# LeiXu84/fireFoam-dev

Measured on AMD Instinct MI355X. Metric: PIMPLE outer-iterations/sec on 64M-cell hex mesh; pEqn SpMV GB/s vs HBM peak, higher is better.
Workload: dtype f64; 1 GPU; synthetic 400^3 hex box (64000000 cells), buoyant plume + 5-species EDC-shaped source, PIMPLE 1/2/0: rhoEqn + UEqn + YEEqn(4 Yi + h) + 2 pEqn per step; cells=64000000, faces=191520000, parallelism=1 GPU, transport_solvers=PBiCGStab+DILU

## Files before the change

### firefoam-dev_amd/binding.py

```python
import ctypes as C
import os
import re
import subprocess

import numpy as np

_HERE = os.path.dirname(os.path.abspath(__file__))
_ROOT = os.path.dirname(_HERE)
_SO = os.path.join(_HERE, "lib", "libffm.so")
_HDR = os.path.join(_ROOT, "include", "ffm.h")

SOLVERS = {"PCG": 0, "PBiCGStab": 1, "PBiCG": 2, "diagonal": 3, "smoothSolver": 4}
PRECONDS = {"none": 0, "DIC": 1, "DILU": 2, "GaussSeidel": 3, "symGaussSeidel": 4, "diagonal": 5}


class FfmError(RuntimeError):
    pass


class Perf(C.Structure):
    _fields_ = [("initialResidual", C.c_double), ("finalResidual", C.c_double),
                ("nIterations", C.c_int), ("converged", C.c_int), ("singular", C.c_int)]

    def as_dict(self):
# ... 62 lines not shown
        "ffm_renumber_levels": ([C.c_int, C.c_int, ip, ip, ip, ip], C.c_int),
        "ffm_ldu_set_coeffs": ([vp, hp, hp, hp], C.c_int),
        "ffm_ldu_set_coeffs_d": ([vp, dp, dp, dp], C.c_int),
        "ffm_ldu_n_native_faces": ([vp], C.c_int),
        "ffm_ldu_get_face_map": ([vp, ip], C.c_int),
        "ffm_ldu_set_coeffs_native_d": ([vp, dp, dp, dp], C.c_int),
        "ffm_ldu_bind_coeffs_native_d": ([vp, dp, dp, dp, C.c_int], C.c_int),
        "ffm_ldu_set_interfaces": ([vp, C.c_int, ip, C.POINTER(ip), C.POINTER(hp), C.POINTER(hp), ip], C.c_int),
        "ffm_ldu_set_global_cells": ([vp, C.c_long], C.c_int),
        "ffm_spmv": ([vp, dp, dp], C.c_int),
        "ffm_tmul": ([vp, dp, dp], C.c_int),
        "ffm_sumA": ([vp, dp], C.c_int),
        "ffm_residual": ([vp, dp, dp, dp], C.c_int),
        "ffm_precond_setup": ([vp, C.c_int, dp], C.c_int),
        "ffm_precond_apply": ([vp, C.c_int, C.c_int, dp, dp], C.c_int),
        "ffm_gs_smooth": ([vp, C.c_int, C.c_int, dp, dp], C.c_int),
        "ffm_solve_d": ([vp, C.c_int, C.c_int, C.c_double, C.c_double, C.c_int, C.c_int, C.c_int, dp, dp,
                         C.POINTER(Perf)], C.c_int),
        "ffm_solve": ([vp, C.c_int, C.c_int, C.c_double, C.c_double, C.c_int, C.c_int, C.c_int, hp, hp,
                       C.POINTER(Perf)], C.c_int),
        "ffm_solve_multi_d": ([vp, C.c_int, C.c_int, C.c_int, C.c_double, C.c_double, C.c_int, C.c_int, C.POINTER(C.c_void_p), dp, dp,
                               C.POINTER(C.c_void_p), C.POINTER(C.c_void_p), C.POINTER(Perf)], C.c_int),
        "ffm_ldu_unbind_coeffs": ([vp], C.c_int),
        "ffm_bench_spmv": ([vp, dp, dp, C.c_int, hp], C.c_int),
        "ffm_bench_precond": ([vp, C.c_int, dp, dp, C.c_int, hp], C.c_int),
        "ffm_debug_set_sweep_ticket": ([vp, C.c_uint], C.c_int),
        "ffm_ldu_set_exchange_tags": ([vp, C.c_int, C.c_int, ip], C.c_int),
        "ffm_field_binary": ([vp, C.c_int, C.c_long, dp, dp, dp], C.c_int),
        "ffm_field_scalar": ([vp, C.c_int, C.c_long, dp, C.c_double, C.c_int, dp], C.c_int),
        "ffm_field_unary": ([vp, C.c_int, C.c_long, dp, dp], C.c_int),
# ... 430 lines not shown

    def residual(self, psi, source):
        self.ctx._ready()
        r = self.ctx.empty(self.nCells)
        _check(lib().ffm_residual(self.h, C.c_void_p(psi.data_ptr()), C.c_void_p(source.data_ptr()),
                                  C.c_void_p(r.data_ptr())), "ffm_residual")
        self.ctx.sync()
        return r

    def reciprocalD(self, preconditioner):
        rD = self.ctx.empty(self.nCells)
        _check(lib().ffm_precond_setup(self.h, PRECONDS[preconditioner], C.c_void_p(rD.data_ptr())), "ffm_precond_setup")
        self.ctx.sync()
        return rD

    def precondition(self, preconditioner, rA, transpose=False):
        self.ctx._ready()
        w = self.ctx.empty(self.nCells)
        _check(lib().ffm_precond_apply(self.h, PRECONDS[preconditioner], 1 if transpose else 0,
                                       C.c_void_p(rA.data_ptr()), C.c_void_p(w.data_ptr())), "ffm_precond_apply")
        self.ctx.sync()
        return w

    def smooth(self, psi, source, nSweeps=1, smoother="symGaussSeidel"):
        self.ctx._ready()
        psi = psi.clone()
        self.ctx._ready()
        _check(lib().ffm_gs_smooth(self.h, 1 if smoother == "symGaussSeidel" else 0, nSweeps,
                                   C.c_void_p(psi.data_ptr()), C.c_void_p(source.data_ptr())), "ffm_gs_smooth")
        self.ctx.sync()
# ... 414 lines not shown
```

### firefoam-dev_amd/csrc/ffm_solve.hip

```cpp
#include "ffm_internal.hpp"
#include "ffm_device.hpp"
#include <algorithm>
#include <cmath>
#include <cstring>

static inline int sgrid(long n) { long g = (n + 255) / 256; return (int)std::max(1L, std::min(g, (long)RED_BLOCKS)); }

enum {
    OP_XREF = 1, OP_NORMF, OP_RES_INIT, OP_RES, OP_PCG_BETA, OP_PCG_ALPHA,
    OP_BS_RHO, OP_BS_ALPHA, OP_BS_OMEGA, OP_BICG_BETA, OP_BICG_ALPHA, OP_RESET
};

#define VSMALL_ 1e-300

__global__ void k_scalar_op(double *__restrict__ s, int op, double arg, int iter)
{
    if (threadIdx.x || blockIdx.x) return;
    switch (op) {
    case OP_RESET:
        s[S_SING] = 0.0; s[S_WARA] = 1e+20; s[S_WARA_OLD] = 1e+20; s[S_RA0RA] = 0.0; s[S_ALPHA] = 0.0; s[S_OMEGA] = 0.0;
        s[S_BETA] = 0.0;
        break;
    case OP_XREF: s[S_XREF] = s[S_TMP0] / arg; break;
    case OP_NORMF: s[S_NORMF] = s[S_TMP0] + 1e-20; break;
    case OP_RES_INIT: s[S_RES] = s[S_TMP0] / s[S_NORMF]; s[S_RES0] = s[S_RES]; break;
    case OP_RES: if (s[S_SING] == 0.0) s[S_RES] = s[S_TMP0] / s[S_NORMF]; break;
    case OP_PCG_BETA: {
        const double old = s[S_WARA], nw = s[S_TMP0];
        s[S_WARA_OLD] = old; s[S_WARA] = nw; s[S_BETA] = nw / old;
        break; }
    case OP_PCG_ALPHA: case OP_BICG_ALPHA: {
        const double wApA = s[S_TMP0];
        s[S_WAPA] = wApA;
        if (fabs(wApA) / s[S_NORMF] > VSMALL_) { s[S_ALPHA] = s[S_WARA] / wApA; }
        else { s[S_SING] = 1.0; s[S_ALPHA] = 0.0; }
        break; }
    case OP_BS_RHO: {
        const double old = s[S_RA0RA], nw = s[S_TMP0];
        s[S_RA0RA_OLD] = old; s[S_RA0RA] = nw;
        if (!(fabs(nw) > VSMALL_)) { s[S_SING] = 1.0; break; }
        if (iter > 0) {
            if (!(fabs(s[S_OMEGA]) > VSMALL_)) { s[S_SING] = 1.0; break; }
            s[S_BETA] = (nw / old) * (s[S_ALPHA] / s[S_OMEGA]);
        }
        break; }
    case OP_BS_ALPHA: if (s[S_SING] == 0.0) { s[S_RA0AYA] = s[S_TMP0]; s[S_ALPHA] = s[S_RA0RA] / s[S_TMP0]; } break;
    case OP_BS_OMEGA: if (s[S_SING] == 0.0) { s[S_TATA] = s[S_TMP0]; s[S_TASA] = s[S_TMP1]; s[S_OMEGA] = s[S_TMP1] / s[S_TMP0]; } break;
    case OP_BICG_BETA: {
        const double old = s[S_WARA], nw = s[S_TMP0];
        s[S_WARA_OLD] = old; s[S_WARA] = nw; s[S_BETA] = nw / old;
        break; }
    }
}

static int scalar_op(ffm_ctx *c, int op, double arg = 0.0, int iter = 0)
{
    hipLaunchKernelGGL(k_scalar_op, dim3(1), dim3(64), 0, c->stream, c->scal_d, op, arg, iter);
    FFM_HIP(hipGetLastError());
    return FFM_OK;
}
static int finish_dot(ffm_ctx *c, int op, int nSlots = 1, double arg = 0.0, int iter = 0)
{
    if (c->nRanks > 1 || c->comm) FFM_TRY(ffm_allreduce_slots(c, S_TMP0, nSlots));
    return scalar_op(c, op, arg, iter);
}

#define GRID_STRIDE(i, n) for (long i = (long)blockIdx.x * blockDim.x + threadIdx.x; i < (n); i += (long)gridDim.x * blockDim.x)

__global__ void k_sub(long n, double *__restrict__ r, const double *__restrict__ b, const double *__restrict__ w)
{ GRID_STRIDE(i, n) r[i] = b[i] - w[i]; }

__global__ void k_sub2(long n, double *__restrict__ r, double *__restrict__ rT, const double *__restrict__ b,
                       const double *__restrict__ w, const double *__restrict__ wT)
{ GRID_STRIDE(i, n) { r[i] = b[i] - w[i]; rT[i] = b[i] - wT[i]; } }

__global__ void k_copy(long n, double *__restrict__ d, const double *__restrict__ s)
{ GRID_STRIDE(i, n) d[i] = s[i]; }

__global__ __launch_bounds__(256) void k_normf(long n, const double *__restrict__ Ax, const double *__restrict__ b,
                                               const double *__restrict__ sumA, const double *__restrict__ scal,
                                               double *__restrict__ partials)
{
    __shared__ double sm[4];
    const double xRef = scal[S_XREF];
    double acc = 0.0;
    GRID_STRIDE(i, n) { const double t = sumA[i] * xRef; acc += fabs(Ax[i] - t) + fabs(b[i] - t); }
    const double r = block_sum(acc, sm);
    if (threadIdx.x == 0) partials[blockIdx.x] = r;
}

__global__ void k_p_update(long n, double *__restrict__ p, const double *__restrict__ w, const double *__restrict__ scal, int first)
{
    if (scal[S_SING] != 0.0) return;
    const double beta = scal[S_BETA];
    if (first) { GRID_STRIDE(i, n) p[i] = w[i]; }
    else { GRID_STRIDE(i, n) p[i] = w[i] + beta * p[i]; }
}

__global__ void k_p_psi(long n, double *__restrict__ psi, double *__restrict__ p, const double *__restrict__ w, const double *__restrict__ scal)
{
    if (scal[S_SING] != 0.0) return;
    const double alpha = scal[S_ALPHA], beta = scal[S_BETA];
    GRID_STRIDE(i, n) { const double pi = p[i]; psi[i] += alpha * pi; p[i] = w[i] + beta * pi; }
// ... 12 lines not shown
        if (!sing) { psi[i] += alpha * p[i]; ri -= alpha * w[i]; r[i] = ri; }
        acc += fabs(ri);
    }
    const double s = block_sum(acc, sm);
    if (threadIdx.x == 0) partials[blockIdx.x] = s;
}

__global__ void k_axmy_alpha(long n, double *__restrict__ r, const double *__restrict__ w, const double *__restrict__ scal)
{
    if (scal[S_SING] != 0.0) return;
    const double alpha = scal[S_ALPHA];
    GRID_STRIDE(i, n) r[i] -= alpha * w[i];
}

__global__ void k_bs_p(long n, double *__restrict__ p, const double *__restrict__ r, const double *__restrict__ AyA,
                       const double *__restrict__ scal, int first)
{
    if (scal[S_SING] != 0.0) return;
    const double beta = scal[S_BETA], omega = scal[S_OMEGA];
    if (first) { GRID_STRIDE(i, n) p[i] = r[i]; }
    else { GRID_STRIDE(i, n) p[i] = r[i] + beta * (p[i] - omega * AyA[i]); }
}

__global__ __launch_bounds__(256) void k_bs_s(long n, double *__restrict__ sA, const double *__restrict__ r,
                                              const double *__restrict__ AyA, const double *__restrict__ scal,
                                              double *__restrict__ partials)
{
    __shared__ double sm[4];
    const double alpha = scal[S_ALPHA];
    const bool sing = scal[S_SING] != 0.0;
    double acc = 0.0;
    if (!sing) GRID_STRIDE(i, n) { const double v = r[i] - alpha * AyA[i]; sA[i] = v; acc += fabs(v); }
    const double s = block_sum(acc, sm);
    if (threadIdx.x == 0) partials[blockIdx.x] = s;
}

// ... 240 lines not shown
    FFM_HIP(hipMemcpyAsync(h, A->sweepTicket, sizeof(h), hipMemcpyDeviceToHost, A->ctx->stream));
    FFM_HIP(hipStreamSynchronize(A->ctx->stream));
    if (h[1]) {
        ffm_set_error(A->sweepMode == 2 ? "tiled sweep timed out waiting for a value of a predecessor group (abort word set)"
                                        : "dataflow sweep timed out waiting for the value of a predecessor cell (abort word set)");
        unsigned int z = 0;
        ffm_h2d(A->ctx, A->sweepTicket + 1, &z, sizeof(z));
        return FFM_ERR_HIP;
    }
    return FFM_OK;
}

static int calc_rD(ffm_ldu *A)
{
    if (A->sweepMode == 2) {
        FFM_TRY(ffm_tile_calc_rD(A));
        hipLaunchKernelGGL(k_recip, dim3(sgrid(A->nOwned)), dim3(256), 0, A->ctx->stream, (long)A->nOwned, A->rD, A->rD);
        FFM_HIP(hipGetLastError());
        return FFM_OK;
    }
    FlowArgs a; FFM_TRY(flow_args(A, SM_RD, a));
    FLOW_LAUNCH(SM_RD, a);
    FFM_HIP(hipGetLastError());
    return FFM_OK;
}

int ffm_precond_setup_i(ffm_ldu *A, int precond)
{
    if (A->rDKind == precond && A->rDEpoch == A->coeffEpoch) return FFM_OK;
    hipStream_t s = A->ctx->stream;
    switch (precond) {
    case FFM_NONE: break;
    case FFM_DIC:
        if (!A->symmetric) { ffm_set_error("DIC needs a symmetric matrix"); return FFM_ERR_UNSUPPORTED; }
// ... 52 lines not shown
        a.bP = bUse; a.psi = psi;
        if (sym) FLOW_LAUNCH(SM_SYMGS, a); else FLOW_LAUNCH(SM_GS, a);
        FFM_HIP(hipGetLastError());
    }
    return FFM_OK;
}

struct Controls { double tol, relTol; int minIter, maxIter, nSweeps; };

static inline bool check_convergence(ffm_perf *p, const Controls &k)
{
    p->converged = (p->finalResidual < k.tol || (k.relTol > 1e-20 && p->finalResidual < k.relTol * p->initialResidual)) ? 1 : 0;
    return p->converged;
}

static int norm_and_initial(ffm_ldu *A, const double *psi, const double *source, const double *Apsi, double *tmp,
                            const double *rA, ffm_perf *perf)
{
    ffm_ctx *c = A->ctx; hipStream_t s = c->stream; const long N = A->nOwned;
    FFM_TRY(ffm_k_sum(c, psi, N, S_TMP0));
    FFM_TRY(finish_dot(c, OP_XREF, 1, (double)A->globalCells));
    const int g = sgrid(N);
    hipLaunchKernelGGL(k_normf, dim3(g), dim3(256), 0, s, N, Apsi, source, tmp, c->scal_d, c->partials_d);
    FFM_TRY(partial_sum_to(c, g, S_TMP0));
    FFM_TRY(finish_dot(c, OP_NORMF));
    FFM_TRY(ffm_k_summag(c, rA, N, S_TMP0));
    FFM_TRY(finish_dot(c, OP_RES_INIT));
    FFM_TRY(ffm_read_scalars(c));
    perf->initialResidual = c->scal_h[S_RES0];
    perf->finalResidual = perf->initialResidual;
    perf->nIterations = 0; perf->singular = 0; perf->converged = 0;
    return FFM_OK;
}

static int pcg(ffm_ldu *A, int precond, const Controls &k, double *psi, const double *source, ffm_perf *perf)
{
    ffm_ctx *c = A->ctx; hipStream_t s = c->stream; const long N = A->nOwned; const int g = sgrid(N);
    double *pA, *wA, *rA;
    FFM_TRY(ffm_ldu_work(A, 1, &pA)); FFM_TRY(ffm_ldu_work(A, 2, &wA)); FFM_TRY(ffm_ldu_work(A, 3, &rA));
    FFM_TRY(scalar_op(c, OP_RESET));
    FFM_TRY(ffm_k_spmv_sumA(A, psi, wA, pA));
    hipLaunchKernelGGL(k_sub, dim3(g), dim3(256), 0, s, N, rA, source, wA);
    FFM_TRY(norm_and_initial(A, psi, source, wA, pA, rA, perf));
    if (k.minIter > 0 || !check_convergence(perf, k)) {
        FFM_TRY(ffm_precond_setup_i(A, precond));
        if (precond == FFM_DIC && A->sweepMode == 2 && ffm_tile_pcg_fusable(A)) {
            const bool fuseP = ffm_tile_amul_pcg_usable(A);
            double *pB = nullptr, *qA = wA;
            if (fuseP) { FFM_TRY(ffm_ldu_work(A, 4, &pB)); FFM_TRY(ffm_ldu_work(A, 5, &qA)); }
            do {
                if (perf->nIterations == 0) {
                    FFM_TRY(ffm_precond_apply_i(A, precond, false, rA, wA));
                    FFM_TRY(ffm_k_dot(c, wA, rA, N, S_TMP0));
                } else FFM_TRY(ffm_tile_pcg_bwd(A, rA, wA, S_TMP0));
                FFM_TRY(finish_dot(c, OP_PCG_BETA));
                if (perf->nIterations == 0) {
                    hipLaunchKernelGGL(k_p_update, dim3(g), dim3(256), 0, s, N, pA, wA, c->scal_d, 1);
// ... 26 lines not shown
            hipLaunchKernelGGL(k_pcg_xr, dim3(g), dim3(256), 0, s, N, psi, rA, pA, wA, c->scal_d, c->partials_d);
            FFM_TRY(partial_sum_to(c, g, S_TMP0));
            FFM_TRY(finish_dot(c, OP_RES));
            FFM_TRY(ffm_read_scalars(c));
            if (c->scal_h[S_SING] != 0.0) { perf->singular = 1; break; }
            perf->finalResidual = c->scal_h[S_RES];
        } while ((++perf->nIterations < k.maxIter && !check_convergence(perf, k)) || perf->nIterations < k.minIter);
    }
    return FFM_OK;
}

static int pbicgstab(ffm_ldu *A, int precond, const Controls &k, double *psi, const double *source, ffm_perf *perf)
{
    ffm_ctx *c = A->ctx; hipStream_t s = c->stream; const long N = A->nOwned; const int g = sgrid(N);
    double *yA, *rA, *pA, *AyA, *sA, *zA, *tA, *rA0;
    FFM_TRY(ffm_ldu_work(A, 1, &pA)); FFM_TRY(ffm_ldu_work(A, 2, &yA)); FFM_TRY(ffm_ldu_work(A, 3, &rA));
    FFM_TRY(scalar_op(c, OP_RESET));
    FFM_TRY(ffm_k_spmv_sumA(A, psi, yA, pA));
    hipLaunchKernelGGL(k_sub, dim3(g), dim3(256), 0, s, N, rA, source, yA);
    FFM_TRY(norm_and_initial(A, psi, source, yA, pA, rA, perf));
    if (k.minIter > 0 || !check_convergence(perf, k)) {
        FFM_TRY(ffm_ldu_work(A, 4, &AyA)); FFM_TRY(ffm_ldu_work(A, 5, &sA)); FFM_TRY(ffm_ldu_work(A, 6, &zA));
        FFM_TRY(ffm_ldu_work(A, 7, &tA)); FFM_TRY(ffm_ldu_work(A, 8, &rA0));
        hipLaunchKernelGGL(k_copy, dim3(g), dim3(256), 0, s, N, rA0, rA);
        FFM_TRY(ffm_precond_setup_i(A, precond));
        do {
            FFM_TRY(ffm_k_dot(c, rA0, rA, N, S_TMP0));
            FFM_TRY(finish_dot(c, OP_BS_RHO, 1, 0.0, perf->nIterations));
            hipLaunchKernelGGL(k_bs_p, dim3(g), dim3(256), 0, s, N, pA, rA, AyA, c->scal_d, perf->nIterations == 0 ? 1 : 0);
            FFM_TRY(ffm_precond_apply_i(A, precond, false, pA, yA));
            FFM_TRY(ffm_k_spmv(A, yA, AyA, false));
            FFM_TRY(ffm_k_dot(c, rA0, AyA, N, S_TMP0));
            FFM_TRY(finish_dot(c, OP_BS_ALPHA));
            hipLaunchKernelGGL(k_bs_s, dim3(g), dim3(256), 0, s, N, sA, rA, AyA, c->scal_d, c->partials_d);
            FFM_TRY(partial_sum_to(c, g, S_TMP0));
            FFM_TRY(finish_dot(c, OP_RES));
            FFM_TRY(ffm_read_scalars(c));
            if (c->scal_h[S_SING] != 0.0) { perf->singular = 1; break; }
            perf->finalResidual = c->scal_h[S_RES];
            if (check_convergence(perf, k)) {
                hipLaunchKernelGGL(k_axpy_alpha, dim3(g), dim3(256), 0, s, N, psi, yA, c->scal_d);
                perf->nIterations++;
                return FFM_OK;
            }
// ... 9 lines not shown
            perf->finalResidual = c->scal_h[S_RES];
        } while ((++perf->nIterations < k.maxIter && !check_convergence(perf, k)) || perf->nIterations < k.minIter);
    }
    return FFM_OK;
}

static int pbicg(ffm_ldu *A, int precond, const Controls &k, double *psi, const double *source, ffm_perf *perf)
{
    ffm_ctx *c = A->ctx; hipStream_t s = c->stream; const long N = A->nOwned; const int g = sgrid(N);
    double *pA, *pT, *wA, *wT, *rA, *rT;
    FFM_TRY(ffm_ldu_work(A, 1, &pA)); FFM_TRY(ffm_ldu_work(A, 2, &wA)); FFM_TRY(ffm_ldu_work(A, 3, &rA));
    FFM_TRY(ffm_ldu_work(A, 4, &pT)); FFM_TRY(ffm_ldu_work(A, 5, &wT)); FFM_TRY(ffm_ldu_work(A, 6, &rT));
    FFM_TRY(scalar_op(c, OP_RESET));
    FFM_TRY(ffm_k_spmv_sumA(A, psi, wA, pA));
    FFM_TRY(ffm_k_spmv(A, psi, wT, true));
    hipLaunchKernelGGL(k_sub2, dim3(g), dim3(256), 0, s, N, rA, rT, source, wA, wT);
    FFM_TRY(norm_and_initial(A, psi, source, wA, pA, rA, perf));
    if (k.minIter > 0 || !check_convergence(perf, k)) {
        FFM_TRY(ffm_precond_setup_i(A, precond));
        do {
            FFM_TRY(ffm_precond_apply_i(A, precond, false, rA, wA));
            FFM_TRY(ffm_precond_apply_i(A, precond, true, rT, wT));
            FFM_TRY(ffm_k_dot(c, wA, rT, N, S_TMP0));
            FFM_TRY(finish_dot(c, OP_BICG_BETA));
            const int first = perf->nIterations == 0 ? 1 : 0;
            hipLaunchKernelGGL(k_p_update, dim3(g), dim3(256), 0, s, N, pA, wA, c->scal_d, first);
            hipLaunchKernelGGL(k_p_update, dim3(g), dim3(256), 0, s, N, pT, wT, c->scal_d, first);
            FFM_TRY(ffm_k_spmv(A, pA, wA, false));
            FFM_TRY(ffm_k_spmv(A, pT, wT, true));
            FFM_TRY(ffm_k_dot(c, wA, pT, N, S_TMP0));
            FFM_TRY(finish_dot(c, OP_BICG_ALPHA));
            hipLaunchKernelGGL(k_axmy_alpha, dim3(g), dim3(256), 0, s, N, rT, wT, c->scal_d);
            hipLaunchKernelGGL(k_pcg_xr, dim3(g), dim3(256), 0, s, N, psi, rA, pA, wA, c->scal_d, c->partials_d);
            FFM_TRY(partial_sum_to(c, g, S_TMP0));
            FFM_TRY(finish_dot(c, OP_RES));
            FFM_TRY(ffm_read_scalars(c));
            if (c->scal_h[S_SING] != 0.0) { perf->singular = 1; break; }
            perf->finalResidual = c->scal_h[S_RES];
        } while ((++perf->nIterations < k.maxIter && !check_convergence(perf, k)) || perf->nIterations < k.minIter);
    }
    return FFM_OK;
}

static int smooth(ffm_ldu *A, int smoother, const Controls &k, double *psi, const double *source, ffm_perf *perf)
{
    if (smoother != FFM_GS && smoother != FFM_SYMGS) { ffm_set_error("smoothSolver: smoother must be GaussSeidel or symGaussSeidel"); return FFM_ERR_UNSUPPORTED; }
    ffm_ctx *c = A->ctx; hipStream_t s = c->stream; const long N = A->nOwned; const int g = sgrid(N);
    const int nSweeps = k.nSweeps > 0 ? k.nSweeps : 1;
    double *Apsi, *tmp, *res;
    FFM_TRY(ffm_ldu_work(A, 1, &Apsi)); FFM_TRY(ffm_ldu_work(A, 2, &tmp)); FFM_TRY(ffm_ldu_work(A, 3, &res));
    FFM_TRY(scalar_op(c, OP_RESET));
    FFM_TRY(ffm_k_spmv_sumA(A, psi, Apsi, tmp));
    hipLaunchKernelGGL(k_sub, dim3(g), dim3(256), 0, s, N, res, source, Apsi);
    FFM_TRY(norm_and_initial(A, psi, source, Apsi, tmp, res, perf));
    if (k.minIter > 0 || !check_convergence(perf, k)) {
        do {
            FFM_TRY(ffm_gs_smooth_i(A, smoother == FFM_SYMGS, nSweeps, psi, source));
            FFM_TRY(ffm_k_residual(A, psi, source, res));
            FFM_TRY(ffm_k_summag(c, res, N, S_TMP0));
            FFM_TRY(finish_dot(c, OP_RES));
            FFM_TRY(ffm_read_scalars(c));
            perf->finalResidual = c->scal_h[S_RES];
        } while (((perf->nIterations += nSweeps) < k.maxIter && !check_convergence(perf, k)) || perf->nIterations < k.minIter);
    }
    return FFM_OK;
}

static int diagonal(ffm_ldu *A, double *psi, const double *source, ffm_perf *perf)
// ... 89 lines not shown
    if (m == 1) { G.use(L[only]); return ffm_k_spmv(A, L[only].*in, L[only].*out, false); }
    return FFM_OK;
}
static int pbicgstab_multi(ffm_ldu *A, int precond, const Controls &k, int n, Lane *L)
{
    ffm_ctx *c = A->ctx; hipStream_t s = c->stream; const long N = A->nOwned; const int g = sgrid(N);
    LaneGuard G(A);
    {
        const double *dg[FFM_TILE_MAXSYS], *x[FFM_TILE_MAXSYS]; double *y[FFM_TILE_MAXSYS], *sm[FFM_TILE_MAXSYS];
        for (int i = 0; i < n; i++) { dg[i] = L[i].diag; x[i] = L[i].psi; y[i] = L[i].yA; sm[i] = L[i].pA; }
        FFM_TRY(ffm_k_spmv_multi(A, n, dg, x, y, sm));
    }
    for (int i = 0; i < n; i++) {
        Lane &l = L[i]; G.use(l);
        FFM_TRY(scalar_op(c, OP_RESET));
        hipLaunchKernelGGL(k_sub, dim3(g), dim3(256), 0, s, N, l.rA, l.source, l.yA);
        FFM_TRY(norm_and_initial(A, l.psi, l.source, l.yA, l.pA, l.rA, l.perf));
        l.active = k.minIter > 0 || !check_convergence(l.perf, k);
        if (l.active) hipLaunchKernelGGL(k_copy, dim3(g), dim3(256), 0, s, N, l.rA0, l.rA);
    }
    {
        const double *dg[FFM_TILE_MAXSYS]; double *D[FFM_TILE_MAXSYS]; int m = 0, only = -1;
        for (int i = 0; i < n; i++) if (L[i].active) { dg[m] = L[i].diag; D[m] = L[i].rD; m++; only = i; }
        if (m >= 2) {
            FFM_TRY(ffm_tile_calc_rD_multi(A, m, dg, D));
            for (int j = 0; j < m; j++) hipLaunchKernelGGL(k_recip, dim3(g), dim3(256), 0, s, N, D[j], (const double *)D[j]);
        } else if (m == 1) { G.use(L[only]); A->rDKind = -1; FFM_TRY(ffm_precond_setup_i(A, precond)); }
        A->rDKind = precond; A->rDEpoch = A->coeffEpoch;
    }
    for (;;) {
        bool any = false;
        for (int i = 0; i < n; i++) if (L[i].active) {
            Lane &l = L[i]; G.use(l); any = true;
            FFM_TRY(ffm_k_dot(c, l.rA0, l.rA, N, S_TMP0));
            FFM_TRY(finish_dot(c, OP_BS_RHO, 1, 0.0, l.perf->nIterations));
            hipLaunchKernelGGL(k_bs_p, dim3(g), dim3(256), 0, s, N, l.pA, l.rA, l.AyA, c->scal_d, l.perf->nIterations == 0 ? 1 : 0);
        }
        if (!any) break;
        FFM_TRY(precond_lanes(A, precond, L, n, &Lane::pA, &Lane::yA, G));
        FFM_TRY(amul_lanes(A, L, n, &Lane::yA, &Lane::AyA, G));
        for (int i = 0; i < n; i++) if (L[i].active) {
            Lane &l = L[i]; G.use(l);
            FFM_TRY(ffm_k_dot(c, l.rA0, l.AyA, N, S_TMP0));
            FFM_TRY(finish_dot(c, OP_BS_ALPHA));
            hipLaunchKernelGGL(k_bs_s, dim3(g), dim3(256), 0, s, N, l.sA, l.rA, l.AyA, c->scal_d, c->partials_d);
            FFM_TRY(partial_sum_to(c, g, S_TMP0));
            FFM_TRY(finish_dot(c, OP_RES));
        }
        FFM_TRY(read_lane_scalars(c, L, n));
        for (int i = 0; i < n; i++) if (L[i].active) {
            Lane &l = L[i]; G.use(l);
// ... 76 lines not shown
    const size_t nb = sizeof(double) * (size_t)std::max(A->nCells, 1);
    FFM_HIP(hipMalloc((void **)&p, nb)); FFM_HIP(hipMalloc((void **)&b, nb));
    FFM_TRY(ffm_h2d(A->ctx, p, psi, sizeof(double) * A->nOwned));
    FFM_TRY(ffm_h2d(A->ctx, b, source, sizeof(double) * A->nOwned));
    int rc = ffm_solve_d(A, solver, precond, tol, relTol, minIter, maxIter, nSweeps, p, b, out);
    if (!rc) rc = ffm_d2h(A->ctx, psi, p, sizeof(double) * A->nOwned);
    hipFree(p); hipFree(b);
    return rc;
}

extern "C" int ffm_precond_setup(ffm_ldu *A, int precond, double *rD_out_d)
{
    if (!A) return FFM_ERR_ARG;
    FFM_TRY(ffm_precond_setup_i(A, precond));
    if (rD_out_d) FFM_TRY(ffm_from_internal(A, A->rD, rD_out_d));
    FFM_HIP(hipStreamSynchronize(A->ctx->stream));
    FFM_TRY(ffm_sweep_check_abort(A));
    return FFM_OK;
}

extern "C" int ffm_bench_precond(ffm_ldu *A, int precond, const double *r_d, double *w_d, int reps, double *avg_ms)
{
    if (!A || !r_d || !w_d || reps < 1 || !avg_ms) return FFM_ERR_ARG;
    if (!A->identity) { ffm_set_error("ffm_bench_precond needs an LDU in the library's cell order"); return FFM_ERR_UNSUPPORTED; }
    FFM_TRY(ffm_precond_setup_i(A, precond));
    FFM_TRY(ffm_precond_apply_i(A, precond, false, r_d, w_d));
    hipEvent_t e0, e1;
    FFM_HIP(hipEventCreate(&e0)); FFM_HIP(hipEventCreate(&e1));
    FFM_HIP(hipEventRecord(e0, A->ctx->stream));
    for (int i = 0; i < reps; i++) FFM_TRY(ffm_precond_apply_i(A, precond, false, r_d, w_d));
// ... 40 lines not shown
```

### firefoam-dev_amd/csrc/ffm_tile.hip

```cpp
#include "ffm_internal.hpp"
#include "ffm_device.hpp"
#include <algorithm>
#include <atomic>
#include <climits>

constexpr int T_RING = 4096;
constexpr int T_ENT = 256;
constexpr int T_THREADS = 256;
constexpr int T_W = 3;
constexpr int T_PF = 8;
constexpr int T_PM = 3;
constexpr int T_XMAX = 64;
constexpr int T_RINGD = T_RING - 2 * T_ENT;
constexpr unsigned T_SPIN_LIMIT = 1u << 22;
constexpr unsigned T_NONE = 0xFFFFu;
constexpr int T_LDS = T_RING + 2 * T_XMAX + 1;
constexpr unsigned long long T_SENT = 0x7FF4DEADBEEFCAFEull;
static_assert(T_LDS < (int)T_NONE && T_ENT <= 256, "neighbour codes are LDS slots");
static_assert(T_PM >= 2 && T_PM < T_PF, "read-ahead distances");

struct TileDir {
    int nEnt = 0, nPub = 0;
    int *grpEnt = nullptr;
    int4 *rec = nullptr;
// ... 447 lines not shown
                    for (int s = 0; s < W; s++) { const double nv = val - pa[k][s] * pb[k][TWO ? s : 0] / x[s]; val = (cd[s] != T_NONE) ? nv : val; }
                } else if (MODE == TM_GSF) {
                    val = pv[k];
#pragma unroll
                    for (int s = 0; s < W; s++) { const double nv = val - pa[k][s] * x[s]; val = (cd[s] != T_NONE) ? nv : val; }
                    if (pok[k]) *(double *)((char *)aux + c * 8u) = val;
#pragma unroll
                    for (int s = 0; s < W; s++) val -= pb[k][TWO ? s : 0];
                    val = val / d;
                } else {
                    val = pv[k];
#pragma unroll
                    for (int s = 0; s < W; s++) { const double nv = val - pa[k][s] * x[s]; val = (cd[s] != T_NONE) ? nv : val; }
                    val = val / d;
                }
                if (pok[k]) { *(double *)((char *)w + c * 8u) = val; ring[(c - gs) & (unsigned)(T_RING - 1)] = val; }
                if (FUSE && MODE == TM_BWD) fsum += pok[k] ? val * pv2[FUSE ? k : 0] : 0.0;
                if (pok[k] && cd[3] != T_NONE) t_st(&t.mail[ppb[k] + cd[3]], val);
            }
            T_FETCH(k, ee + T_PF, Rn);
            t_barrier();
        }
    }
#undef T_FETCH
    if (FUSE) {
        double v = fsum;
#pragma unroll
        for (int o = 32; o > 0; o >>= 1) v += __shfl_down(v, o, 64);
        if ((tid & 63u) == 0u) shSum[tid >> 6] = v;
        t_barrier();
        if (tid == 0) partials[g] = ((shSum[0] + shSum[1]) + shSum[2]) + shSum[3];
// ... 247 lines not shown
                        for (int s = 0; s < W; s++) { const double nv = v - d * pa[k][s] * ring[i][sl[s]]; v = (cd[s] != T_NONE) ? nv : v; }
                    } else if (MODE == TM_BWD) {
                        v = pv[k][TWO ? 0 : i];
#pragma unroll
                        for (int s = W - 1; s >= 0; s--) { const double nv = v - d * pa[k][s] * ring[i][sl[s]]; v = (cd[s] != T_NONE) ? nv : v; }
                    } else {
                        v = d;
#pragma unroll
                        for (int s = 0; s < W; s++) { const double nv = v - pa[k][s] * pb[k][TWO ? s : 0] / ring[i][sl[s]]; v = (cd[s] != T_NONE) ? nv : v; }
                    }
                    val[i] = v;
                }
                if (pok[k]) {
#pragma unroll
                    for (int i = 0; i < NF; i++) {
                        *(double *)((char *)m.w[i] + c * 8u) = val[i];
                        ring[i][(c - gs) & (unsigned)(T_RING - 1)] = val[i];
                        if (cd[3] != T_NONE) t_st(&m.mail[i][ppb[k] + cd[3]], val[i]);
                    }
                }
            }
            TM_FETCH(k, ee + PF, Rn);
            t_barrier();
        }
    }
#undef TM_FETCH
}


bool ffm_tile_multi_usable(const ffm_ldu *A) { return ffm_tile_usable(A); }
static int tile_multi_mail(ffm_ldu *A)
// ... 308 lines not shown
```

### include/ffm.h

```cpp
#ifndef FFM_H
#define FFM_H

#include <stddef.h>
#include <stdint.h>

#ifdef __cplusplus
extern "C" {
#endif

typedef struct ffm_ctx ffm_ctx;
typedef struct ffm_ldu ffm_ldu;

typedef enum ffm_status {
    FFM_OK = 0,
    FFM_ERR_ARG = -1,
    FFM_ERR_ADDR = -2,
    FFM_ERR_HIP = -3,
    FFM_ERR_NODEVICE = -4,
    FFM_ERR_UNSUPPORTED = -5,
    FFM_ERR_COMM = -6
} ffm_status;

typedef enum ffm_solver {
    FFM_PCG = 0, FFM_PBICGSTAB = 1, FFM_PBICG = 2, FFM_DIAGONAL = 3, FFM_SMOOTH = 4,
// ... 81 lines not shown
int ffm_ldu_set_interfaces(ffm_ldu *ldu, int nPatches, const int *patchSizes,
                           const int *const *faceCells,
                           const double *const *bouCoeffs,
                           const double *const *intCoeffs,
                           const int *neighbRank);
int ffm_ldu_set_global_cells(ffm_ldu *ldu, long globalCells);
int ffm_ldu_set_exchange_tags(ffm_ldu *ldu, int kind, int n, const int *tags);

int ffm_spmv(ffm_ldu *ldu, const double *x_d, double *y_d);
int ffm_tmul(ffm_ldu *ldu, const double *x_d, double *y_d);
int ffm_sumA(ffm_ldu *ldu, double *s_d);
int ffm_residual(ffm_ldu *ldu, const double *x_d, const double *b_d, double *r_d);
int ffm_precond_setup(ffm_ldu *ldu, int precond, double *rD_out_d );
int ffm_precond_apply(ffm_ldu *ldu, int precond, int transpose,
                      const double *r_d, double *w_d);
int ffm_gs_smooth(ffm_ldu *ldu, int symmetric_sweep, int nSweeps, double *psi_d,
                  const double *b_d);

int ffm_solve_d(ffm_ldu *ldu, int solver, int precond, double tolerance,
                double relTol, int minIter, int maxIter, int nSweeps,
                double *psi_d, const double *source_d, ffm_perf *out);
int ffm_solve(ffm_ldu *ldu, int solver, int precond, double tolerance,
              double relTol, int minIter, int maxIter, int nSweeps,
              double *psi, const double *source, ffm_perf *out);
int ffm_solve_multi_d(ffm_ldu *ldu, int nSys, int solver, int precond, double tolerance, double relTol, int minIter, int maxIter,
                      const double *const *diag_d, const double *upper_d, const double *lower_d, double *const *psi_d,
                      const double *const *source_d, ffm_perf *out );

int ffm_bench_spmv(ffm_ldu *ldu, const double *x_d, double *y_d, int reps,
                   double *avg_ms);
// ... 249 lines not shown
```

Before: 2.823 outer-iterations/s.

## Fuse solver prologue residual, norm and BiCGStab init; fold reciprocal into tiled rD sweep

Replaces the separate residual subtraction, normalisation-factor reduction, residual-magnitude reduction, r0 copy and first-iteration p copy with a single prologue kernel. It computes r = b - Ax, writes r0 and p, and produces three block partial sums in one pass. The first BiCGStab iteration takes rho from the fused r·r sum instead of launching a dot product. The tiled rD sweep now stores 1/d directly, which removes the separate reciprocal kernels, and a multi-system rD setup entry point is exposed. The aim is fewer launches and fewer full-vector memory passes per solve, at the cost of more register pressure in the prologue and a changed rD contract that must match every consumer.

```diff
diff --git a/firefoam-dev_amd/binding.py b/firefoam-dev_amd/binding.py
--- a/firefoam-dev_amd/binding.py
+++ b/firefoam-dev_amd/binding.py
@@ -100,6 +100,7 @@
         "ffm_residual": ([vp, dp, dp, dp], C.c_int),
         "ffm_precond_setup": ([vp, C.c_int, dp], C.c_int),
         "ffm_precond_apply": ([vp, C.c_int, C.c_int, dp, dp], C.c_int),
+        "ffm_precond_setup_multi": ([vp, C.c_int, C.c_int, C.POINTER(C.c_void_p), C.POINTER(C.c_void_p)], C.c_int),
         "ffm_gs_smooth": ([vp, C.c_int, C.c_int, dp, dp], C.c_int),
         "ffm_solve_d": ([vp, C.c_int, C.c_int, C.c_double, C.c_double, C.c_int, C.c_int, C.c_int, dp, dp,
                          C.POINTER(Perf)], C.c_int),
@@ -560,6 +561,15 @@
         self.ctx.sync()
         return rD
 
+    def reciprocalD_multi(self, preconditioner, diags):
+        self.ctx._ready()
+        n = len(diags)
+        out = [self.ctx.empty(self.nCells) for _ in range(n)]
+        arr = lambda ts: (C.c_void_p * n)(*[t.data_ptr() for t in ts])
+        _check(lib().ffm_precond_setup_multi(self.h, PRECONDS[preconditioner], n, arr(diags), arr(out)), "ffm_precond_setup_multi")
+        self.ctx.sync()
+        return out
+
     def precondition(self, preconditioner, rA, transpose=False):
         self.ctx._ready()
         w = self.ctx.empty(self.nCells)
diff --git a/firefoam-dev_amd/csrc/ffm_solve.hip b/firefoam-dev_amd/csrc/ffm_solve.hip
--- a/firefoam-dev_amd/csrc/ffm_solve.hip
+++ b/firefoam-dev_amd/csrc/ffm_solve.hip
@@ -13,7 +13,7 @@
 
 #define VSMALL_ 1e-300
 
-__global__ void k_scalar_op(double *__restrict__ s, int op, double arg, int iter)
+__global__ void k_scalar_op(double *__restrict__ s, int op, double arg, int iter, int in)
 {
     if (threadIdx.x || blockIdx.x) return;
     switch (op) {
@@ -23,7 +23,7 @@
         break;
     case OP_XREF: s[S_XREF] = s[S_TMP0] / arg; break;
     case OP_NORMF: s[S_NORMF] = s[S_TMP0] + 1e-20; break;
-    case OP_RES_INIT: s[S_RES] = s[S_TMP0] / s[S_NORMF]; s[S_RES0] = s[S_RES]; break;
+    case OP_RES_INIT: s[S_RES] = s[in] / s[S_NORMF]; s[S_RES0] = s[S_RES]; break;
     case OP_RES: if (s[S_SING] == 0.0) s[S_RES] = s[S_TMP0] / s[S_NORMF]; break;
     case OP_PCG_BETA: {
         const double old = s[S_WARA], nw = s[S_TMP0];
@@ -36,7 +36,7 @@
         else { s[S_SING] = 1.0; s[S_ALPHA] = 0.0; }
         break; }
     case OP_BS_RHO: {
-        const double old = s[S_RA0RA], nw = s[S_TMP0];
+        const double old = s[S_RA0RA], nw = s[in];
         s[S_RA0RA_OLD] = old; s[S_RA0RA] = nw;
         if (!(fabs(nw) > VSMALL_)) { s[S_SING] = 1.0; break; }
         if (iter > 0) {
@@ -53,9 +53,9 @@
     }
 }
 
-static int scalar_op(ffm_ctx *c, int op, double arg = 0.0, int iter = 0)
-{
-    hipLaunchKernelGGL(k_scalar_op, dim3(1), dim3(64), 0, c->stream, c->scal_d, op, arg, iter);
+static int scalar_op(ffm_ctx *c, int op, double arg = 0.0, int iter = 0, int in = S_TMP0)
+{
+    hipLaunchKernelGGL(k_scalar_op, dim3(1), dim3(64), 0, c->stream, c->scal_d, op, arg, iter, in);
     FFM_HIP(hipGetLastError());
     return FFM_OK;
 }
@@ -70,23 +70,33 @@
 __global__ void k_sub(long n, double *__restrict__ r, const double *__restrict__ b, const double *__restrict__ w)
 { GRID_STRIDE(i, n) r[i] = b[i] - w[i]; }
 
-__global__ void k_sub2(long n, double *__restrict__ r, double *__restrict__ rT, const double *__restrict__ b,
-                       const double *__restrict__ w, const double *__restrict__ wT)
-{ GRID_STRIDE(i, n) { r[i] = b[i] - w[i]; rT[i] = b[i] - wT[i]; } }
 
 __global__ void k_copy(long n, double *__restrict__ d, const double *__restrict__ s)
 { GRID_STRIDE(i, n) d[i] = s[i]; }
 
-__global__ __launch_bounds__(256) void k_normf(long n, const double *__restrict__ Ax, const double *__restrict__ b,
-                                               const double *__restrict__ sumA, const double *__restrict__ scal,
-                                               double *__restrict__ partials)
+template <bool BS>
+__global__ __launch_bounds__(256) void k_prologue(long n, const double *__restrict__ Ax, const double *__restrict__ b, const double *sumA,
+                                                  const double *__restrict__ scal, double *__restrict__ r, double *__restrict__ r0,
+                                                  double *p, double *__restrict__ partials)
 {
     __shared__ double sm[4];
     const double xRef = scal[S_XREF];
-    double acc = 0.0;
-    GRID_STRIDE(i, n) { const double t = sumA[i] * xRef; acc += fabs(Ax[i] - t) + fabs(b[i] - t); }
-    const double r = block_sum(acc, sm);
-    if (threadIdx.x == 0) partials[blockIdx.x] = r;
+    double accN = 0.0, accR = 0.0, accD = 0.0;
+    GRID_STRIDE(i, n) {
+        const double ax = Ax[i], bi = b[i], t = sumA[i] * xRef;
+        const double ri = bi - ax;
+        accN += fabs(ax - t) + fabs(bi - t);
+        accR += fabs(ri);
+        r[i] = ri;
+        if (BS) { accD += ri * ri; r0[i] = ri; p[i] = ri; }
+    }
+    const double sN = block_sum(accN, sm);
+    const double sR = block_sum(accR, sm);
+    const double sD = BS ? block_sum(accD, sm) : 0.0;
+    if (threadIdx.x == 0) {
+        partials[blockIdx.x] = sN; partials[RED_BLOCKS + blockIdx.x] = sR;
+        if (BS) partials[2 * RED_BLOCKS + blockIdx.x] = sD;
+    }
 }
 
 __global__ void k_p_update(long n, double *__restrict__ p, const double *__restrict__ w, const double *__restrict__ scal, int first)
@@ -129,12 +139,11 @@
 }
 
 __global__ void k_bs_p(long n, double *__restrict__ p, const double *__restrict__ r, const double *__restrict__ AyA,
-                       const double *__restrict__ scal, int first)
+                       const double *__restrict__ scal)
 {
     if (scal[S_SING] != 0.0) return;
     const double beta = scal[S_BETA], omega = scal[S_OMEGA];
-    if (first) { GRID_STRIDE(i, n) p[i] = r[i]; }
-    else { GRID_STRIDE(i, n) p[i] = r[i] + beta * (p[i] - omega * AyA[i]); }
+    GRID_STRIDE(i, n) p[i] = r[i] + beta * (p[i] - omega * AyA[i]);
 }
 
 __global__ __launch_bounds__(256) void k_bs_s(long n, double *__restrict__ sA, const double *__restrict__ r,
@@ -405,10 +414,7 @@
 static int calc_rD(ffm_ldu *A)
 {
     if (A->sweepMode == 2) {
-        FFM_TRY(ffm_tile_calc_rD(A));
-        hipLaunchKernelGGL(k_recip, dim3(sgrid(A->nOwned)), dim3(256), 0, A->ctx->stream, (long)A->nOwned, A->rD, A->rD);
-        FFM_HIP(hipGetLastError());
-        return FFM_OK;
+        return ffm_tile_calc_rD(A);
     }
     FlowArgs a; FFM_TRY(flow_args(A, SM_RD, a));
     FLOW_LAUNCH(SM_RD, a);
@@ -491,18 +497,18 @@
     return p->converged;
 }
 
-static int norm_and_initial(ffm_ldu *A, const double *psi, const double *source, const double *Apsi, double *tmp,
-                            const double *rA, ffm_perf *perf)
+static int norm_and_initial(ffm_ldu *A, const double *psi, const double *source, const double *Apsi, const double *tmp,
+                            double *rA, ffm_perf *perf, double *rA0 = nullptr, double *pA = nullptr)
 {
     ffm_ctx *c = A->ctx; hipStream_t s = c->stream; const long N = A->nOwned;
     FFM_TRY(ffm_k_sum(c, psi, N, S_TMP0));
     FFM_TRY(finish_dot(c, OP_XREF, 1, (double)A->globalCells));
-    const int g = sgrid(N);
-    hipLaunchKernelGGL(k_normf, dim3(g), dim3(256), 0, s, N, Apsi, source, tmp, c->scal_d, c->partials_d);
-    FFM_TRY(partial_sum_to(c, g, S_TMP0));
-    FFM_TRY(finish_dot(c, OP_NORMF));
-    FFM_TRY(ffm_k_summag(c, rA, N, S_TMP0));
-    FFM_TRY(finish_dot(c, OP_RES_INIT));
+    const int g = sgrid(N), nSums = rA0 ? 3 : 2;
+    if (rA0) hipLaunchKernelGGL(k_prologue<true>, dim3(g), dim3(256), 0, s, N, Apsi, source, tmp, c->scal_d, rA, rA0, pA, c->partials_d);
+    else hipLaunchKernelGGL(k_prologue<false>, dim3(g), dim3(256), 0, s, N, Apsi, source, tmp, c->scal_d, rA, (double *)nullptr, (double *)nullptr, c->partials_d);
+    FFM_TRY(partial_sum_to(c, g, S_TMP0, nSums));
+    FFM_TRY(finish_dot(c, OP_NORMF, nSums));
+    FFM_TRY(scalar_op(c, OP_RES_INIT, 0.0, 0, S_TMP1));
     FFM_TRY(ffm_read_scalars(c));
     perf->initialResidual = c->scal_h[S_RES0];
     perf->finalResidual = perf->initialResidual;
@@ -517,7 +523,6 @@
     FFM_TRY(ffm_ldu_work(A, 1, &pA)); FFM_TRY(ffm_ldu_work(A, 2, &wA)); FFM_TRY(ffm_ldu_work(A, 3, &rA));
     FFM_TRY(scalar_op(c, OP_RESET));
     FFM_TRY(ffm_k_spmv_sumA(A, psi, wA, pA));
-    hipLaunchKernelGGL(k_sub, dim3(g), dim3(256), 0, s, N, rA, source, wA);
     FFM_TRY(norm_and_initial(A, psi, source, wA, pA, rA, perf));
     if (k.minIter > 0 || !check_convergence(perf, k)) {
         FFM_TRY(ffm_precond_setup_i(A, precond));
@@ -574,20 +579,21 @@
 {
     ffm_ctx *c = A->ctx; hipStream_t s = c->stream; const long N = A->nOwned; const int g = sgrid(N);
     double *yA, *rA, *pA, *AyA, *sA, *zA, *tA, *rA0;
-    FFM_TRY(ffm_ldu_work(A, 1, &pA)); FFM_TRY(ffm_ldu_work(A, 2, &yA)); FFM_TRY(ffm_ldu_work(A, 3, &rA));
+    FFM_TRY(ffm_ldu_work(A, 1, &pA)); FFM_TRY(ffm_ldu_work(A, 2, &yA)); FFM_TRY(ffm_ldu_work(A, 3, &rA)); FFM_TRY(ffm_ldu_work(A, 8, &rA0));
     FFM_TRY(scalar_op(c, OP_RESET));
     FFM_TRY(ffm_k_spmv_sumA(A, psi, yA, pA));
-    hipLaunchKernelGGL(k_sub, dim3(g), dim3(256), 0, s, N, rA, source, yA);
-    FFM_TRY(norm_and_initial(A, psi, source, yA, pA, rA, perf));
+    FFM_TRY(norm_and_initial(A, psi, source, yA, pA, rA, perf, rA0, pA));
     if (k.minIter > 0 || !check_convergence(perf, k)) {
         FFM_TRY(ffm_ldu_work(A, 4, &AyA)); FFM_TRY(ffm_ldu_work(A, 5, &sA)); FFM_TRY(ffm_ldu_work(A, 6, &zA));
-        FFM_TRY(ffm_ldu_work(A, 7, &tA)); FFM_TRY(ffm_ldu_work(A, 8, &rA0));
-        hipLaunchKernelGGL(k_copy, dim3(g), dim3(256), 0, s, N, rA0, rA);
+        FFM_TRY(ffm_ldu_work(A, 7, &tA));
         FFM_TRY(ffm_precond_setup_i(A, precond));
         do {
-            FFM_TRY(ffm_k_dot(c, rA0, rA, N, S_TMP0));
-            FFM_TRY(finish_dot(c, OP_BS_RHO, 1, 0.0, perf->nIterations));
-            hipLaunchKernelGGL(k_bs_p, dim3(g), dim3(256), 0, s, N, pA, rA, AyA, c->scal_d, perf->nIterations == 0 ? 1 : 0);
+            if (perf->nIterations == 0) FFM_TRY(scalar_op(c, OP_BS_RHO, 0.0, 0, S_TMP2));
+            else {
+                FFM_TRY(ffm_k_dot(c, rA0, rA, N, S_TMP0));
+                FFM_TRY(finish_dot(c, OP_BS_RHO, 1, 0.0, perf->nIterations));
+                hipLaunchKernelGGL(k_bs_p, dim3(g), dim3(256), 0, s, N, pA, rA, AyA, c->scal_d);
+            }
             FFM_TRY(ffm_precond_apply_i(A, precond, false, pA, yA));
             FFM_TRY(ffm_k_spmv(A, yA, AyA, false));
             FFM_TRY(ffm_k_dot(c, rA0, AyA, N, S_TMP0));
@@ -627,7 +633,7 @@
     FFM_TRY(scalar_op(c, OP_RESET));
     FFM_TRY(ffm_k_spmv_sumA(A, psi, wA, pA));
     FFM_TRY(ffm_k_spmv(A, psi, wT, true));
-    hipLaunchKernelGGL(k_sub2, dim3(g), dim3(256), 0, s, N, rA, rT, source, wA, wT);
+    hipLaunchKernelGGL(k_sub, dim3(g), dim3(256), 0, s, N, rT, source, wT);
     FFM_TRY(norm_and_initial(A, psi, source, wA, pA, rA, perf));
     if (k.minIter > 0 || !check_convergence(perf, k)) {
         FFM_TRY(ffm_precond_setup_i(A, precond));
@@ -658,13 +664,12 @@
 static int smooth(ffm_ldu *A, int smoother, const Controls &k, double *psi, const double *source, ffm_perf *perf)
 {
     if (smoother != FFM_GS && smoother != FFM_SYMGS) { ffm_set_error("smoothSolver: smoother must be GaussSeidel or symGaussSeidel"); return FFM_ERR_UNSUPPORTED; }
-    ffm_ctx *c = A->ctx; hipStream_t s = c->stream; const long N = A->nOwned; const int g = sgrid(N);
+    ffm_ctx *c = A->ctx; const long N = A->nOwned;
     const int nSweeps = k.nSweeps > 0 ? k.nSweeps : 1;
     double *Apsi, *tmp, *res;
     FFM_TRY(ffm_ldu_work(A, 1, &Apsi)); FFM_TRY(ffm_ldu_work(A, 2, &tmp)); FFM_TRY(ffm_ldu_work(A, 3, &res));
     FFM_TRY(scalar_op(c, OP_RESET));
     FFM_TRY(ffm_k_spmv_sumA(A, psi, Apsi, tmp));
-    hipLaunchKernelGGL(k_sub, dim3(g), dim3(256), 0, s, N, res, source, Apsi);
     FFM_TRY(norm_and_initial(A, psi, source, Apsi, tmp, res, perf));
     if (k.minIter > 0 || !check_convergence(perf, k)) {
         do {
@@ -784,27 +789,24 @@
     for (int i = 0; i < n; i++) {
         Lane &l = L[i]; G.use(l);
         FFM_TRY(scalar_op(c, OP_RESET));
-        hipLaunchKernelGGL(k_sub, dim3(g), dim3(256), 0, s, N, l.rA, l.source, l.yA);
-        FFM_TRY(norm_and_initial(A, l.psi, l.source, l.yA, l.pA, l.rA, l.perf));
+        FFM_TRY(norm_and_initial(A, l.psi, l.source, l.yA, l.pA, l.rA, l.perf, l.rA0, l.pA));
         l.active = k.minIter > 0 || !check_convergence(l.perf, k);
-        if (l.active) hipLaunchKernelGGL(k_copy, dim3(g), dim3(256), 0, s, N, l.rA0, l.rA);
     }
     {
         const double *dg[FFM_TILE_MAXSYS]; double *D[FFM_TILE_MAXSYS]; int m = 0, only = -1;
         for (int i = 0; i < n; i++) if (L[i].active) { dg[m] = L[i].diag; D[m] = L[i].rD; m++; only = i; }
-        if (m >= 2) {
-            FFM_TRY(ffm_tile_calc_rD_multi(A, m, dg, D));
-            for (int j = 0; j < m; j++) hipLaunchKernelGGL(k_recip, dim3(g), dim3(256), 0, s, N, D[j], (const double *)D[j]);
-        } else if (m == 1) { G.use(L[only]); A->rDKind = -1; FFM_TRY(ffm_precond_setup_i(A, precond)); }
+        if (m >= 2) FFM_TRY(ffm_tile_calc_rD_multi(A, m, dg, D));
+        else if (m == 1) { G.use(L[only]); A->rDKind = -1; FFM_TRY(ffm_precond_setup_i(A, precond)); }
         A->rDKind = precond; A->rDEpoch = A->coeffEpoch;
     }
     for (;;) {
         bool any = false;
         for (int i = 0; i < n; i++) if (L[i].active) {
             Lane &l = L[i]; G.use(l); any = true;
+            if (l.perf->nIterations == 0) { FFM_TRY(scalar_op(c, OP_BS_RHO, 0.0, 0, S_TMP2)); continue; }
             FFM_TRY(ffm_k_dot(c, l.rA0, l.rA, N, S_TMP0));
             FFM_TRY(finish_dot(c, OP_BS_RHO, 1, 0.0, l.perf->nIterations));
-            hipLaunchKernelGGL(k_bs_p, dim3(g), dim3(256), 0, s, N, l.pA, l.rA, l.AyA, c->scal_d, l.perf->nIterations == 0 ? 1 : 0);
+            hipLaunchKernelGGL(k_bs_p, dim3(g), dim3(256), 0, s, N, l.pA, l.rA, l.AyA, c->scal_d);
         }
         if (!any) break;
         FFM_TRY(precond_lanes(A, precond, L, n, &Lane::pA, &Lane::yA, G));
@@ -911,6 +913,20 @@
     if (!A) return FFM_ERR_ARG;
     FFM_TRY(ffm_precond_setup_i(A, precond));
     if (rD_out_d) FFM_TRY(ffm_from_internal(A, A->rD, rD_out_d));
+    FFM_HIP(hipStreamSynchronize(A->ctx->stream));
+    FFM_TRY(ffm_sweep_check_abort(A));
+    return FFM_OK;
+}
+
+extern "C" int ffm_precond_setup_multi(ffm_ldu *A, int precond, int nSys, const double *const *diag_d, double *const *rD_out_d)
+{
+    if (!A || !diag_d || !rD_out_d || nSys < 2 || nSys > FFM_TILE_MAXSYS) { ffm_set_error("ffm_precond_setup_multi: bad argument"); return FFM_ERR_ARG; }
+    if (precond != FFM_DIC && precond != FFM_DILU) { ffm_set_error("ffm_precond_setup_multi: DIC or DILU"); return FFM_ERR_UNSUPPORTED; }
+    if (!(A->identity && A->sweepMode == 2 && ffm_tile_multi_usable(A))) { ffm_set_error("ffm_precond_setup_multi needs a tiled matrix in the library's cell order"); return FFM_ERR_UNSUPPORTED; }
+    if (precond == FFM_DIC && !A->symmetric) { ffm_set_error("DIC needs a symmetric matrix"); return FFM_ERR_UNSUPPORTED; }
+    for (int i = 0; i < nSys; i++) if (!diag_d[i] || !rD_out_d[i]) { ffm_set_error("ffm_precond_setup_multi: null array"); return FFM_ERR_ARG; }
+    FFM_HIP(hipSetDevice(A->ctx->device));
+    FFM_TRY(ffm_tile_calc_rD_multi(A, nSys, diag_d, rD_out_d));
     FFM_HIP(hipStreamSynchronize(A->ctx->stream));
     FFM_TRY(ffm_sweep_check_abort(A));
     return FFM_OK;
diff --git a/firefoam-dev_amd/csrc/ffm_tile.hip b/firefoam-dev_amd/csrc/ffm_tile.hip
--- a/firefoam-dev_amd/csrc/ffm_tile.hip
+++ b/firefoam-dev_amd/csrc/ffm_tile.hip
@@ -485,7 +485,7 @@
                     for (int s = 0; s < W; s++) { const double nv = val - pa[k][s] * x[s]; val = (cd[s] != T_NONE) ? nv : val; }
                     val = val / d;
                 }
-                if (pok[k]) { *(double *)((char *)w + c * 8u) = val; ring[(c - gs) & (unsigned)(T_RING - 1)] = val; }
+                if (pok[k]) { *(double *)((char *)w + c * 8u) = (MODE == TM_RD) ? 1.0 / val : val; ring[(c - gs) & (unsigned)(T_RING - 1)] = val; }
                 if (FUSE && MODE == TM_BWD) fsum += pok[k] ? val * pv2[FUSE ? k : 0] : 0.0;
                 if (pok[k] && cd[3] != T_NONE) t_st(&t.mail[ppb[k] + cd[3]], val);
             }
@@ -763,7 +763,7 @@
                 if (pok[k]) {
 #pragma unroll
                     for (int i = 0; i < NF; i++) {
-                        *(double *)((char *)m.w[i] + c * 8u) = val[i];
+                        *(double *)((char *)m.w[i] + c * 8u) = (MODE == TM_RD) ? 1.0 / val[i] : val[i];
                         ring[i][(c - gs) & (unsigned)(T_RING - 1)] = val[i];
                         if (cd[3] != T_NONE) t_st(&m.mail[i][ppb[k] + cd[3]], val[i]);
                     }
diff --git a/include/ffm.h b/include/ffm.h
--- a/include/ffm.h
+++ b/include/ffm.h
@@ -119,6 +119,7 @@
 int ffm_precond_setup(ffm_ldu *ldu, int precond, double *rD_out_d );
 int ffm_precond_apply(ffm_ldu *ldu, int precond, int transpose,
                       const double *r_d, double *w_d);
+int ffm_precond_setup_multi(ffm_ldu *ldu, int precond, int nSys, const double *const *diag_d, double *const *rD_out_d);
 int ffm_gs_smooth(ffm_ldu *ldu, int symmetric_sweep, int nSweeps, double *psi_d,
                   const double *b_d);
 
```

Measured after the change: 2.882 outer-iterations/s (median of 6 runs). 2.1% higher.
